# microsoft/hyperspace

Measured on NVIDIA H100. Metric: createIndex rows/sec, higher is better.
Workload: dtype int64

## Files before the change

### hyperspace_b200/csrc/radix_sort.cu

```cuda
#include <cmath>

#include "device_utils.cuh"
#include "kernels.h"

namespace hs {

struct SortChunk {
  uint32_t seg;
  uint32_t tile_begin, tile_end;
};

namespace {

constexpr int kThreads = 512;
constexpr int kWarps = kThreads / 32;
constexpr int kItems = kSortTile / kThreads;
constexpr int kWarpRows = kSortTile / kWarps;
constexpr int kChunkTiles = 128;
constexpr int kHistThreads = 256;

struct DigitShift {
  int shift;
  __device__ __forceinline__ uint32_t operator()(uint64_t key, uint32_t) const { return (uint32_t)(key >> shift) & 255u; }
};
struct DigitTable {
  const uint8_t* table;
  __device__ __forceinline__ uint32_t operator()(uint64_t, uint32_t val) const { return table[val]; }
};

struct SrcPairs {
  const uint64_t* __restrict__ keys;
  const uint32_t* __restrict__ vals;
  __device__ __forceinline__ void load(uint64_t p, uint64_t& k, uint32_t& v) const {
    k = keys[p];
    v = vals[p];
  }
};
template <int TYPE>
struct SrcRaw {
  const void* __restrict__ raw;
  __device__ __forceinline__ void load(uint64_t p, uint64_t& k, uint32_t& v) const {
    const uint64_t r = (TYPE == HS_TYPE_INT64 || TYPE == HS_TYPE_DOUBLE) ? ((const uint64_t*)raw)[p]
                                                                          : (uint64_t)((const uint32_t*)raw)[p];
    k = sort_encode(TYPE, r);
    v = (uint32_t)p;
  }
};

template <typename Src, typename Digit>
__global__ void __launch_bounds__(kHistThreads) k_sort_hist(const SortTile* __restrict__ tiles, Src src, Digit digit,
                                                         uint32_t* __restrict__ tile_hist) {
  __shared__ uint32_t s_hist[256];
  s_hist[threadIdx.x] = 0;
  __syncthreads();
  const SortTile t = tiles[blockIdx.x];
  for (uint32_t i = threadIdx.x; i < t.count; i += kHistThreads) {
    uint64_t k;
    uint32_t v;
    src.load(t.start + i, k, v);
    atomicAdd(&s_hist[digit(k, v)], 1u);
  }
  __syncthreads();
  tile_hist[(size_t)blockIdx.x * 256 + threadIdx.x] = s_hist[threadIdx.x];
}

__global__ void __launch_bounds__(256) k_seg_chunk_sums(const SortChunk* __restrict__ chunks,
                                                         const uint32_t* __restrict__ tile_hist,
                                                         uint32_t* __restrict__ chunk_sums) {
  const SortChunk c = chunks[blockIdx.x];
  uint32_t s = 0;
  for (uint32_t t = c.tile_begin; t < c.tile_end; t++) s += tile_hist[(size_t)t * 256 + threadIdx.x];
  chunk_sums[(size_t)blockIdx.x * 256 + threadIdx.x] = s;
}

__global__ void __launch_bounds__(256) k_seg_scan(const uint32_t* __restrict__ seg_chunk_begin,
                                                   const uint64_t* __restrict__ seg_start,
                                                   uint32_t* __restrict__ chunk_sums, uint32_t* __restrict__ digit_base) {
  __shared__ uint32_t warp_sums[40];
  const uint32_t seg = blockIdx.x;
  const uint32_t c0 = seg_chunk_begin[seg], c1 = seg_chunk_begin[seg + 1];
  uint32_t tot = 0;
  for (uint32_t c = c0; c < c1; c++) {
    const uint32_t v = chunk_sums[(size_t)c * 256 + threadIdx.x];
    chunk_sums[(size_t)c * 256 + threadIdx.x] = tot;
    tot += v;
  }
  const uint32_t dbase = block_exclusive_scan(tot, warp_sums, nullptr) + (uint32_t)seg_start[seg];
  if (digit_base) digit_base[(size_t)seg * 256 + threadIdx.x] = dbase;
  for (uint32_t c = c0; c < c1; c++) chunk_sums[(size_t)c * 256 + threadIdx.x] += dbase;
}

__global__ void __launch_bounds__(1024) k_seg_apply(const SortChunk* __restrict__ chunks,
                                                     const uint32_t* __restrict__ tile_hist,
                                                     uint32_t* __restrict__ tile_dst,
                                                     const uint32_t* __restrict__ chunk_sums) {
  __shared__ uint32_t s_group[4][256];
  const SortChunk c = chunks[blockIdx.x];
  const uint32_t d = threadIdx.x & 255, g = threadIdx.x >> 8;
  const uint32_t n = c.tile_end - c.tile_begin;
  const uint32_t per = (n + 3) / 4;
  const uint32_t t0 = c.tile_begin + min(g * per, n), t1 = c.tile_begin + min((g + 1) * per, n);
  uint32_t s = 0;
#pragma unroll 8
  for (uint32_t t = t0; t < t1; t++) s += tile_hist[(size_t)t * 256 + d];
  s_group[g][d] = s;
  __syncthreads();
  uint32_t run = chunk_sums[(size_t)blockIdx.x * 256 + d];
  for (uint32_t gg = 0; gg < g; gg++) run += s_group[gg][d];
#pragma unroll 8
  for (uint32_t t = t0; t < t1; t++) {
    const uint32_t v = tile_hist[(size_t)t * 256 + d];
    tile_dst[(size_t)t * 256 + d] = run;
    run += v;
  }
}

template <int W, int I, bool kGuard, typename Bin>
__device__ __forceinline__ uint32_t rank_tile(uint16_t (&cnt)[W][256], uint32_t* warp_sums, Bin bin, uint32_t count,
                                              uint32_t (&rank)[I]) {
  const uint32_t warp = threadIdx.x >> 5, lane = threadIdx.x & 31;
  const unsigned lt = (1u << lane) - 1;
  uint16_t* wcnt = cnt[warp];
#pragma unroll
  for (int j = 0; j < I; j++) {
    rank[j] = 0;
    if (!kGuard || warp * (I * 32) + j * 32 < count) {
      const uint32_t b = bin(j);
      const unsigned peers = match_any_full<8>(b);
      const uint32_t before = __popc(peers & lt);
      const uint32_t pre = wcnt[b];
      __syncwarp();
      if (before == 0) wcnt[b] = (uint16_t)(pre + __popc(peers));
      __syncwarp();
      rank[j] = pre + before;
    }
  }
  __syncthreads();
  uint32_t total = 0;
  if (threadIdx.x < 256) {
#pragma unroll
    for (int w = 0; w < W; w++) total += cnt[w][threadIdx.x];
  }
  const uint32_t start = block_exclusive_scan(total, warp_sums, nullptr);
  if (threadIdx.x < 256) {
    uint32_t run = start;
#pragma unroll
    for (int w = 0; w < W; w++) {
      const uint16_t c = cnt[w][threadIdx.x];
      cnt[w][threadIdx.x] = (uint16_t)run;
      run += c;
    }
  }
  return start;
}

struct ScatterShared {
  uint64_t keys[kSortTile];
  uint32_t vals[kSortTile];
  uint16_t cnt[kWarps][256];
  uint32_t out_adj[256];
  uint32_t warp_sums[40];
};

template <typename Src, typename Digit>
__global__ void __launch_bounds__(kThreads, 2) k_sort_scatter(const SortTile* __restrict__ tiles, Src src, Digit digit,
                                                               const uint32_t* __restrict__ tile_dst,
                                                               uint64_t* __restrict__ out_keys,
                                                               uint32_t* __restrict__ out_vals) {
  extern __shared__ __align__(16) uint8_t smem_raw[];
  ScatterShared& sm = *reinterpret_cast<ScatterShared*>(smem_raw);
  const uint32_t warp = threadIdx.x >> 5, lane = threadIdx.x & 31;
  {
    uint32_t* z = reinterpret_cast<uint32_t*>(&sm.cnt[0][0]);
#pragma unroll
    for (int i = 0; i < kWarps * 256 / 2 / kThreads; i++) z[threadIdx.x + i * kThreads] = 0;
  }
  const SortTile t = tiles[blockIdx.x];
  uint32_t dst0 = 0;
  if (threadIdx.x < 256) dst0 = tile_dst[(size_t)blockIdx.x * 256 + threadIdx.x];
  const uint32_t first = warp * kWarpRows + lane;
  const uint64_t p0 = t.start + first;
  uint64_t k[kItems];
  uint32_t v[kItems];
  uint32_t bin[kItems];
#pragma unroll
  for (int j = 0; j < kItems; j++) {
    const bool a = first + j * 32 < t.count;
    k[j] = ~0ull;
    v[j] = 0;
    if (a) src.load(p0 + j * 32, k[j], v[j]);
    bin[j] = a ? digit(k[j], v[j]) : 255u;
  }
  __syncthreads();
  uint32_t rank[kItems];
  const uint32_t start = rank_tile<kWarps, kItems, false>(sm.cnt, sm.warp_sums, [&](int j) { return bin[j]; }, 0, rank);
  if (threadIdx.x < 256) sm.out_adj[threadIdx.x] = dst0 - start;
  __syncthreads();
  const uint16_t* cnt = sm.cnt[warp];
#pragma unroll
  for (int j = 0; j < kItems; j++) {
    const uint32_t pos = cnt[bin[j]] + rank[j];
    sm.keys[pos] = k[j];
    sm.vals[pos] = v[j];
  }
  __syncthreads();
#pragma unroll
  for (int j = 0; j < kItems; j++) {
    const uint32_t i = threadIdx.x + j * kThreads;
    if (i < t.count) {
      const uint64_t key = sm.keys[i];
      const uint32_t val = sm.vals[i];
      const uint32_t dst = sm.out_adj[digit(key, val)] + i;
      out_keys[dst] = key;
      out_vals[dst] = val;
    }
  }
}

constexpr uint32_t kFixMaxRun = 64;
__global__ void __launch_bounds__(256) k_fix_runs(const SortTile* __restrict__ tiles, const uint64_t* __restrict__ seg_start,
                                                   uint64_t* __restrict__ keys, uint32_t* __restrict__ vals,
                                                   uint64_t high_mask, uint64_t low_mask, uint32_t max_run,
                                                   uint32_t* __restrict__ flag) {
  __shared__ uint64_t s_key[kSortTile + 2];
  __shared__ uint16_t s_heads[kSortTile / 2], s_len[kSortTile / 2];
  const SortTile t = tiles[blockIdx.x];
  const uint64_t segb = seg_start[t.seg], sege = seg_start[t.seg + 1];
  const unsigned lane = threadIdx.x & 31, lt = (1u << lane) - 1;
  constexpr int kPer = kSortTile / 256;
  {
    uint64_t k[kPer];
#pragma unroll
    for (int j = 0; j < kPer; j++) {
      const uint32_t i = j * 256 + threadIdx.x;
      k[j] = i < t.count ? keys[t.start + i] : 0;
    }
#pragma unroll
    for (int j = 0; j < kPer; j++) s_key[1 + j * 256 + threadIdx.x] = k[j];
  }
  __syncthreads();
  if (threadIdx.x == 0) {
    const uint64_t flip = high_mask & (~high_mask + 1);
    s_key[0] = t.start > segb ? keys[t.start - 1] : (s_key[1] ^ flip);
    s_key[t.count + 1] = t.start + t.count < sege ? keys[t.start + t.count] : (s_key[t.count] ^ flip);
  }
  __syncthreads();
  const uint32_t wid = threadIdx.x >> 5;
  uint16_t* my_heads = s_heads + wid * (kSortTile / 16);
  uint16_t* my_len = s_len + wid * (kSortTile / 16);
  uint32_t my_n = 0;
#pragma unroll 4
  for (uint32_t i0 = 0; i0 < kSortTile; i0 += 256) {
    const uint32_t i = i0 + threadIdx.x;
    bool head = false;
    if (i < t.count) {
      const uint64_t kh = s_key[1 + i] & high_mask;
      head = (s_key[i] & high_mask) != kh && (s_key[2 + i] & high_mask) == kh;
    }
    const unsigned m = __ballot_sync(0xffffffffu, head);
    if (head) my_heads[my_n + __popc(m & lt)] = (uint16_t)i;
    my_n += __popc(m);
  }
  __syncwarp();
  for (uint32_t e = lane; e < my_n; e += 32) {
    const uint32_t i = my_heads[e];
    const uint64_t* sk = s_key + 1 + i;
    const uint64_t kh = sk[0] & high_mask;
    uint32_t len = 1;
    while (i + len < t.count && len <= max_run && (sk[len] & high_mask) == kh) len++;
    const bool crosses = i + len == t.count && (sk[len] & high_mask) == kh;
    my_len[e] = crosses ? (uint16_t)0xffffu : (uint16_t)len;
  }
  __syncthreads();
  for (uint32_t e = lane; e < my_n; e += 32) {
    const uint32_t i = my_heads[e];
    const uint64_t p = t.start + i;
    uint64_t* sk = s_key + 1 + i;
    const uint64_t kh = sk[0] & high_mask;
    uint32_t len = my_len[e];
    if (len == 0xffffu) {
      len = t.count - i;
      uint64_t q = p + len;
      while (q < sege && q - p <= max_run && (keys[q] & high_mask) == kh) q++;
      const uint32_t glen = (uint32_t)(q - p);
      if (glen > max_run) {
        *flag = 1;
        continue;
      }
      for (uint32_t a = 1; a < glen; a++) {
        const uint64_t ka = keys[p + a];
        const uint32_t va = vals[p + a];
        const uint64_t la = ka & low_mask;
        uint32_t b = a;
        while (b > 0 && (keys[p + b - 1] & low_mask) > la) {
          keys[p + b] = keys[p + b - 1];
          vals[p + b] = vals[p + b - 1];
          b--;
        }
        if (b != a) {
          keys[p + b] = ka;
          vals[p + b] = va;
        }
      }
      continue;
    }
    if (len > max_run) {
      *flag = 1;
      continue;
    }
    for (uint32_t a = 1; a < len; a++) {
      const uint64_t ka = sk[a];
      const uint64_t la = ka & low_mask;
      uint32_t b = a;
      while (b > 0 && (sk[b - 1] & low_mask) > la) b--;
      if (b == a) continue;
      const uint32_t va = vals[p + a];
      for (uint32_t c = a; c > b; c--) {
        const uint64_t kc = sk[c - 1];
        sk[c] = kc;
        keys[p + c] = kc;
        vals[p + c] = vals[p + c - 1];
      }
      sk[b] = ka;
      keys[p + b] = ka;
      vals[p + b] = va;
    }
  }
}

constexpr int kLocalSortCap = 12288;
struct LocalSortItem {
  uint32_t start, count;
};
constexpr int kLocalThreads = 1024;
constexpr int kLocalWarps = kLocalThreads / 32;
constexpr int kLocalItems = kLocalSortCap / kLocalThreads;
constexpr int kLocalWarpRows = kLocalSortCap / kLocalWarps;
constexpr uint32_t kLocalMaxRun = 64;
static_assert(kLocalSortCap % kLocalThreads == 0 && kLocalSortCap <= 65536, "slot numbers are 16-bit");

struct LocalShared {
  uint64_t keys[kLocalSortCap];
  uint32_t vals[kLocalSortCap];
  uint16_t slot[kLocalSortCap];
  uint16_t cnt[kLocalWarps][256];
  uint32_t warp_sums[40];
  unsigned long long or_bits, and_bits;
  uint32_t long_run;
};

__device__ __forceinline__ void local_pass(LocalShared& sm, uint32_t count, int shift) {
  const uint32_t warp = threadIdx.x >> 5, lane = threadIdx.x & 31;
  {
    uint32_t* z = reinterpret_cast<uint32_t*>(&sm.cnt[0][0]);
#pragma unroll
    for (int i = 0; i < kLocalWarps * 256 / 2 / kLocalThreads; i++) z[threadIdx.x + i * kLocalThreads] = 0;
  }
  const uint32_t first = warp * kLocalWarpRows + lane;
  uint32_t slot_bin[kLocalItems], rank[kLocalItems];
#pragma unroll
  for (int j = 0; j < kLocalItems; j++) {
    const uint32_t pos = first + j * 32;
    const uint32_t s = pos < count ? sm.slot[pos] : pos;
    slot_bin[j] = s << 8 | (pos < count ? (uint32_t)(sm.keys[s] >> shift) & 255u : 255u);
  }
  __syncthreads();
  rank_tile<kLocalWarps, kLocalItems, true>(sm.cnt, sm.warp_sums, [&](int j) { return slot_bin[j] & 255u; }, count, rank);
  __syncthreads();
  const uint16_t* cnt = sm.cnt[warp];
#pragma unroll
  for (int j = 0; j < kLocalItems; j++)
    if (warp * kLocalWarpRows + j * 32 < count) sm.slot[cnt[slot_bin[j] & 255u] + rank[j]] = (uint16_t)(slot_bin[j] >> 8);
  __syncthreads();
}

template <typename Src>
__global__ void __launch_bounds__(kLocalThreads, 1) k_local_sort(const LocalSortItem* __restrict__ items, Src src,
                                                                 uint64_t* __restrict__ out_keys,
                                                                 uint32_t* __restrict__ out_vals) {
  extern __shared__ __align__(16) uint8_t smem_raw[];
  LocalShared& sm = *reinterpret_cast<LocalShared*>(smem_raw);
  const LocalSortItem it = items[blockIdx.x];
  const uint32_t count = it.count;
  if (threadIdx.x == 0) {
    sm.or_bits = 0;
    sm.and_bits = ~0ull;
    sm.long_run = 0;
  }
  uint64_t k_or = 0, k_and = ~0ull;
  constexpr int kHalf = kLocalItems / 2;
#pragma unroll 1
  for (int h = 0; h < 2; h++) {
    uint64_t k[kHalf];
    uint32_t v[kHalf];
#pragma unroll
    for (int j = 0; j < kHalf; j++) {
      const uint32_t i = (h * kHalf + j) * kLocalThreads + threadIdx.x;
      if (i < count) src.load((uint64_t)it.start + i, k[j], v[j]);
    }
#pragma unroll
    for (int j = 0; j < kHalf; j++) {
      const uint32_t i = (h * kHalf + j) * kLocalThreads + threadIdx.x;
      if (i < count) {
        sm.keys[i] = k[j];
        sm.vals[i] = v[j];
        sm.slot[i] = (uint16_t)i;
        k_or |= k[j];
        k_and &= k[j];
      }
    }
  }
#pragma unroll
  for (int o = 16; o > 0; o >>= 1) {
    k_or |= __shfl_xor_sync(0xffffffffu, k_or, o);
    k_and &= __shfl_xor_sync(0xffffffffu, k_and, o);
  }
  __syncthreads();
  if ((threadIdx.x & 31) == 0) {
    atomicOr(&sm.or_bits, k_or);
    atomicAnd(&sm.and_bits, k_and);
  }
  __syncthreads();
  const uint64_t varying = sm.or_bits ^ sm.and_bits;
  if (varying != 0) {
    const int top = 63 - __clzll((long long)varying);
    int pbits = 1;
    while ((1u << pbits) < 2 * count) pbits++;
    const int ndig = (min(pbits, top + 1) + 7) / 8;
    const int low = max(0, top + 1 - 8 * ndig);
    for (int d = ndig - 1; d >= 0; d--) {
      const int shift = max(0, top + 1 - 8 * (d + 1));
      if ((varying >> shift) & 0xff) local_pass(sm, count, shift);
    }
    const uint64_t high_mask = ~0ull << low;
    if (varying & ~high_mask) {
      for (uint32_t i = threadIdx.x; i < count; i += kLocalThreads) {
        const uint64_t kh = sm.keys[sm.slot[i]] & high_mask;
        if (i > 0 && (sm.keys[sm.slot[i - 1]] & high_mask) == kh) continue;
        if (i + 1 >= count || (sm.keys[sm.slot[i + 1]] & high_mask) != kh) continue;
        uint32_t len = 2;
        while (i + len < count && len <= kLocalMaxRun && (sm.keys[sm.slot[i + len]] & high_mask) == kh) len++;
        if (len > kLocalMaxRun) {
          sm.long_run = 1;
          continue;
        }
        uint16_t* s = sm.slot + i;
        for (uint32_t a = 1; a < len; a++) {
          const uint16_t sa = s[a];
          const uint64_t ka = sm.keys[sa];
          uint32_t b = a;
          while (b > 0 && sm.keys[s[b - 1]] > ka) {
            s[b] = s[b - 1];
            b--;
          }
          s[b] = sa;
        }
      }
      __syncthreads();
      if (sm.long_run) {
        for (uint32_t i = threadIdx.x; i < count; i += kLocalThreads) sm.slot[i] = (uint16_t)i;
        __syncthreads();
        for (int shift = 0; shift < 64; shift += 8)
          if ((varying >> shift) & 0xff) local_pass(sm, count, shift);
      }
    }
  }
  __syncthreads();
#pragma unroll
  for (int j = 0; j < kLocalItems; j++) {
    const uint32_t i = j * kLocalThreads + threadIdx.x;
    if (i < count) {
      const uint32_t s = sm.slot[i];
      out_keys[(uint64_t)it.start + i] = sm.keys[s];
      out_vals[(uint64_t)it.start + i] = sm.vals[s];
    }
  }
}

template <typename Src>
void launch_local_sort(hs_ctx* ctx, const std::vector<LocalSortItem>& items, Src src, uint64_t* out_keys,
                       uint32_t* out_vals) {
  if (items.empty()) return;
  Buf<LocalSortItem> d_items(ctx, items.size());
  copy_h2d(ctx, d_items.get(), items.data(), items.size() * sizeof(LocalSortItem));
  static DeviceOnce attr_once;
  bool& attr = attr_once(ctx->device);
  if (!attr) {
    HS_CUDA(cudaFuncSetAttribute(k_local_sort<Src>, cudaFuncAttributeMaxDynamicSharedMemorySize, (int)sizeof(LocalShared)));
    attr = true;
  }
  KernelScope _ks(ctx, "k_local_sort");
  k_local_sort<Src><<<(unsigned)items.size(), kLocalThreads, sizeof(LocalShared), ctx->stream>>>(d_items.get(), src,
                                                                                                 out_keys, out_vals);
  HS_LAUNCH_CHECK(ctx);
}

template <typename Src, typename Digit>
void run_hist(hs_ctx* ctx, SortPlan* plan, Src src, Digit digit, uint32_t* digit_base) {
  {
    KernelScope _ks(ctx, "k_sort_hist");
    k_sort_hist<Src, Digit><<<(unsigned)plan->ntiles, kHistThreads, 0, ctx->stream>>>(plan->tiles.get(), src, digit,
                                                                                 plan->tile_hist.get());
    HS_LAUNCH_CHECK(ctx);
  }
  KernelScope _ks(ctx, "k_seg_scan");
  k_seg_chunk_sums<<<(unsigned)plan->nchunks, 256, 0, ctx->stream>>>(plan->chunks.get(), plan->tile_hist.get(),
                                                                     plan->chunk_sums.get());
  HS_LAUNCH_CHECK(ctx);
  k_seg_scan<<<(unsigned)plan->nseg, 256, 0, ctx->stream>>>(plan->seg_chunk_begin.get(), plan->seg_start.get(),
                                                            plan->chunk_sums.get(), digit_base);
  HS_LAUNCH_CHECK(ctx);
}

template <typename Src, typename Digit>
void run_scatter(hs_ctx* ctx, SortPlan* plan, Src src, Digit digit, uint64_t* out_keys, uint32_t* out_vals) {
  {
    KernelScope _ks(ctx, "k_seg_scan");
    k_seg_apply<<<(unsigned)plan->nchunks, 1024, 0, ctx->stream>>>(plan->chunks.get(), plan->tile_hist.get(),
                                                                   plan->tile_dst.get(), plan->chunk_sums.get());
    HS_LAUNCH_CHECK(ctx);
  }
  static DeviceOnce attr_once;
  bool& attr = attr_once(ctx->device);
  if (!attr) {
    HS_CUDA(cudaFuncSetAttribute(k_sort_scatter<Src, Digit>, cudaFuncAttributeMaxDynamicSharedMemorySize,
                                 (int)sizeof(ScatterShared)));
    attr = true;
  }
  KernelScope _ks(ctx, "k_sort_scatter");
  k_sort_scatter<Src, Digit><<<(unsigned)plan->ntiles, kThreads, sizeof(ScatterShared), ctx->stream>>>(
      plan->tiles.get(), src, digit, plan->tile_dst.get(), out_keys, out_vals);
  HS_LAUNCH_CHECK(ctx);
}

template <typename Src, typename Digit>
void run_pass(hs_ctx* ctx, SortPlan* plan, Src src, Digit digit, SortedRows* s) {
  run_hist(ctx, plan, src, digit, nullptr);
  run_scatter(ctx, plan, src, digit, s->keys_buf[s->cur ^ 1].get(), s->perm_buf[s->cur ^ 1].get());
  s->cur ^= 1;
}

template <typename F>
void with_raw_source(const KeyColumn& raw, F&& f) {
  switch (raw.type) {
    case HS_TYPE_INT32: f(SrcRaw<HS_TYPE_INT32>{raw.data}); break;
    case HS_TYPE_INT64: f(SrcRaw<HS_TYPE_INT64>{raw.data}); break;
    case HS_TYPE_FLOAT: f(SrcRaw<HS_TYPE_FLOAT>{raw.data}); break;
    case HS_TYPE_DOUBLE: f(SrcRaw<HS_TYPE_DOUBLE>{raw.data}); break;
    default: fail(HS_EUNSUPPORTED, "sort: key type %d", raw.type);
  }
}

void lsd_passes(hs_ctx* ctx, SortPlan* plan, SortedRows* s, uint64_t bits, const KeyColumn* raw) {
  if (plan->ntiles == 0) return;
  bool first = raw != nullptr;
  for (int pass = 0; pass < 8; pass++) {
    if (((bits >> (pass * 8)) & 0xff) == 0) continue;
    const DigitShift digit{pass * 8};
    if (first)
      with_raw_source(*raw, [&](auto src) { run_pass(ctx, plan, src, digit, s); });
    else
      run_pass(ctx, plan, SrcPairs{s->keys(), s->perm()}, digit, s);
    first = false;
  }
  if (first) fail(HS_EINVAL, "sort: raw first-pass source given but no pass ran");
}

void local_sort_segments(hs_ctx* ctx, const SortPlan& plan, const KeyColumn& raw, SortedRows* s) {
  std::vector<LocalSortItem> items;
  for (int g = 0; g < plan.nseg; g++) {
    const uint64_t n = plan.h_seg_start[g + 1] - plan.h_seg_start[g];
    if (n) items.push_back(LocalSortItem{(uint32_t)plan.h_seg_start[g], (uint32_t)n});
  }
  with_raw_source(raw, [&](auto src) { launch_local_sort(ctx, items, src, s->keys(), s->perm()); });
}

bool msd_local_sort(hs_ctx* ctx, SortPlan* plan, const KeyColumn& raw, int shift, SortedRows* s) {
  if (plan->ntiles == 0) return false;
  const size_t nsub = (size_t)plan->nseg * 256;
  Buf<uint32_t> d_base(ctx, nsub);
  const DigitShift digit{shift};
  with_raw_source(raw, [&](auto src) { run_hist(ctx, plan, src, digit, d_base.get()); });
  std::vector<uint32_t> base(nsub + 1);
  copy_d2h(ctx, base.data(), d_base.get(), nsub * 4);
  sync_stream(ctx);
  base[nsub] = (uint32_t)plan->n;
  std::vector<LocalSortItem> items;
  for (int g = 0; g < plan->nseg; g++) {
    LocalSortItem cur{base[(size_t)g * 256], 0};
    for (size_t d = (size_t)g * 256; d < (size_t)(g + 1) * 256; d++) {
      const uint32_t sz = base[d + 1] - base[d];
      if (sz > (uint32_t)kLocalSortCap) return false;
      if (cur.count + sz > (uint32_t)kLocalSortCap) {
        items.push_back(cur);
        cur = LocalSortItem{base[d], 0};
      }
      cur.count += sz;
    }
    if (cur.count) items.push_back(cur);
  }
  uint64_t* keys_alt = s->keys_buf[s->cur ^ 1].get();
  uint32_t* perm_alt = s->perm_buf[s->cur ^ 1].get();
  with_raw_source(raw, [&](auto src) { run_scatter(ctx, plan, src, digit, keys_alt, perm_alt); });
  launch_local_sort(ctx, items, SrcPairs{keys_alt, perm_alt}, s->keys(), s->perm());
  return true;
}

}

__global__ void k_build_tiles(const uint64_t* __restrict__ seg_start, const uint32_t* __restrict__ seg_tile_begin,
                              SortTile* __restrict__ tiles) {
  const uint32_t s = blockIdx.x;
  const uint64_t b = seg_start[s], e = seg_start[s + 1];
  const uint32_t t0 = seg_tile_begin[s], nt = seg_tile_begin[s + 1] - t0;
  for (uint32_t i = threadIdx.x; i < nt; i += blockDim.x) {
    const uint64_t p = b + (uint64_t)i * kSortTile;
    tiles[t0 + i] = SortTile{s, (uint32_t)min((uint64_t)kSortTile, e - p), p};
  }
}

void build_sort_plan(hs_ctx* ctx, const uint64_t* seg_offsets, int nseg, SortPlan* plan) {
  std::vector<uint32_t> stb(nseg + 1), scb(nseg + 1);
  std::vector<uint64_t> sstart(nseg + 1);
  std::vector<SortChunk> chunks;
  uint64_t ntiles = 0;
  for (int s = 0; s < nseg; s++) {
    stb[s] = (uint32_t)ntiles;
    sstart[s] = seg_offsets[s];
    ntiles += ceil_div(seg_offsets[s + 1] - seg_offsets[s], (uint64_t)kSortTile);
    scb[s] = (uint32_t)chunks.size();
    for (uint32_t t = stb[s]; t < ntiles; t += kChunkTiles)
      chunks.push_back(SortChunk{(uint32_t)s, t, (uint32_t)std::min<uint64_t>(t + kChunkTiles, ntiles)});
  }
  stb[nseg] = (uint32_t)ntiles;
  sstart[nseg] = seg_offsets[nseg];
  scb[nseg] = (uint32_t)chunks.size();
  if (seg_offsets[nseg] >= (1ull << 32)) fail(HS_EUNSUPPORTED, "more than 2^32-1 rows per GPU per call");
  plan->n = (int64_t)seg_offsets[nseg];
  plan->ntiles = (int64_t)ntiles;
  plan->nseg = nseg;
  plan->nchunks = (int64_t)chunks.size();
  plan->tiles.alloc(ctx, std::max<size_t>(1, ntiles));
  plan->seg_tile_begin.alloc(ctx, stb.size());
  plan->seg_start.alloc(ctx, sstart.size());
  plan->tile_hist.alloc(ctx, std::max<size_t>(1, ntiles) * 256);
  plan->tile_dst.alloc(ctx, std::max<size_t>(1, ntiles) * 256);
  plan->chunks.alloc(ctx, std::max<size_t>(1, chunks.size()));
  plan->seg_chunk_begin.alloc(ctx, scb.size());
  plan->chunk_sums.alloc(ctx, std::max<size_t>(1, chunks.size()) * 256);
  copy_h2d(ctx, plan->seg_tile_begin.get(), stb.data(), stb.size() * 4);
  copy_h2d(ctx, plan->seg_start.get(), sstart.data(), sstart.size() * 8);
  if (!chunks.empty()) copy_h2d(ctx, plan->chunks.get(), chunks.data(), chunks.size() * sizeof(SortChunk));
  copy_h2d(ctx, plan->seg_chunk_begin.get(), scb.data(), scb.size() * 4);
  if (nseg > 0 && ntiles > 0) {
    k_build_tiles<<<nseg, 256, 0, ctx->stream>>>(plan->seg_start.get(), plan->seg_tile_begin.get(), plan->tiles.get());
    HS_LAUNCH_CHECK(ctx);
  }
  plan->h_seg_tile_begin = std::move(stb);
  plan->h_seg_start = std::move(sstart);
}

void sort_rows(hs_ctx* ctx, SortPlan* plan, const KeyColumn* cols, int ncols, const unsigned long long* last_or_and,
               bool may_defer, SortedRows* out) {
  const int64_t nrows = plan->n;
  for (auto& b : out->keys_buf) b.alloc(ctx, std::max<int64_t>(1, nrows));
  for (auto& b : out->perm_buf) b.alloc(ctx, std::max<int64_t>(1, nrows));
  out->cur = 0;
  out->queued = false;
  out->resort_bits = 0;
  Buf<unsigned long long> d_or_and(ctx, 2);
  unsigned long long or_and[2] = {0, 0};
  auto reduce = [&](auto launch) {
    const unsigned long long init[2] = {0ull, ~0ull};
    copy_h2d(ctx, d_or_and.get(), init, sizeof init);
    launch(d_or_and.get());
    copy_d2h(ctx, or_and, d_or_and.get(), sizeof or_and);
    sync_stream(ctx);
  };
  uint64_t max_seg = 1;
  for (int g = 0; g < plan->nseg; g++) max_seg = std::max<uint64_t>(max_seg, plan->h_seg_start[g + 1] - plan->h_seg_start[g]);
  int want_bytes = 2;
  while (want_bytes < 8 && (double)max_seg / std::pow(256.0, want_bytes) > 0.5) want_bytes++;
  const bool lsd_only = getenv("HS_LSD_SORT") != nullptr;
  for (int k = ncols - 1; k >= 0; k--) {
    const KeyColumn& kc = cols[k];
    const bool from_raw = k == ncols - 1 && kc.type >= HS_TYPE_INT32 && kc.type <= HS_TYPE_DOUBLE;
    if (k == ncols - 1 && !from_raw) launch_iota_u32(ctx, out->perm(), nrows);
    if (kc.type == HS_TYPE_STRING) {
      auto sort_piece = [&](int piece) {
        reduce([&](unsigned long long* d) {
          launch_string_piece_keys(ctx, (const uint64_t*)kc.data, out->perm(), nrows, piece, out->keys(), d);
        });
        lsd_passes(ctx, plan, out, or_and[0] ^ or_and[1], nullptr);
      };
      sort_piece(-1);
      const unsigned long long len_or = or_and[0];
      for (int piece = (int)((len_or + 7) / 8) - 1; piece >= 0; piece--) sort_piece(piece);
    } else {
      if (from_raw && last_or_and) {
        or_and[0] = last_or_and[0];
        or_and[1] = last_or_and[1];
      } else {
        reduce([&](unsigned long long* d) {
          launch_encode_keys(ctx, kc.data, kc.type, from_raw ? nullptr : out->perm(), nrows, from_raw ? nullptr : out->keys(), d);
        });
      }
      const uint64_t varying = nrows ? (or_and[0] ^ or_and[1]) : 0;
      int nbytes = 0, lowest_high_byte = 0;
      for (int b = 7, seen = 0; b >= 0; b--)
        if ((varying >> (8 * b)) & 0xff) {
          nbytes++;
          if (++seen == want_bytes) lowest_high_byte = b;
        }
      const KeyColumn* raw = from_raw ? &kc : nullptr;
      if (from_raw && varying == 0) {
        launch_iota_u32(ctx, out->perm(), nrows);
        launch_encode_keys(ctx, kc.data, kc.type, nullptr, nrows, out->keys(), d_or_and.get());
        raw = nullptr;
      }
      const bool defer = may_defer && ncols == 1 && !kc.valid;
      bool local = false;
      if (raw && !kc.valid && !lsd_only) {
        if (max_seg <= (uint64_t)kLocalSortCap) {
          local_sort_segments(ctx, *plan, kc, out);
          local = true;
        } else if (nbytes > 2 && max_seg <= (uint64_t)(0.85 * 256 * kLocalSortCap)) {
          local = msd_local_sort(ctx, plan, kc, std::max(0, 63 - __builtin_clzll(varying) - 7), out);
        }
      }
      if (local) {
        out->queued = defer;
      } else if (nbytes > want_bytes) {
        const uint64_t high_mask = ~0ull << (8 * lowest_high_byte);
        lsd_passes(ctx, plan, out, varying & high_mask, raw);
        Buf<uint32_t> d_gave_up(ctx, 1);
        fill_bytes(ctx, d_gave_up.get(), 0, 4);
        {
          KernelScope _ks(ctx, "k_fix_runs");
          k_fix_runs<<<(unsigned)plan->ntiles, 256, 0, ctx->stream>>>(plan->tiles.get(), plan->seg_start.get(), out->keys(),
                                                                      out->perm(), high_mask, ~high_mask, kFixMaxRun,
                                                                      d_gave_up.get());
          HS_LAUNCH_CHECK(ctx);
        }
        out->gave_up = 0;
        out->resort_bits = varying;
        out->queued_at = ctx->sync_count;
        out->queued = true;
        copy_d2h(ctx, &out->gave_up, d_gave_up.get(), 4);
        if (!defer) settle_sorted_rows(ctx, plan, out);
      } else {
        lsd_passes(ctx, plan, out, varying, raw);
      }
    }
    if (kc.valid && plan->ntiles)
      run_pass(ctx, plan, SrcPairs{out->keys(), out->perm()}, DigitTable{kc.valid}, out);
  }
}

bool settle_sorted_rows(hs_ctx* ctx, SortPlan* plan, SortedRows* s) {
  const uint64_t bits = s->resort_bits;
  s->queued = false;
  s->resort_bits = 0;
  if (bits == 0) return false;
  if (ctx->sync_count <= s->queued_at) sync_stream(ctx);
  if (!s->gave_up) return false;
  lsd_passes(ctx, plan, s, bits, nullptr);
  return true;
}

}
```

Baseline: 7.955 billion.

## Make local sort persistent with L2 bulk prefetch of next segment

Converts k_local_sort into a persistent kernel with one block per SM looping over items, and uses cp.async.bulk.prefetch.L2 to pull the next item's keys into L2 while the current one sorts. It also loads all items in one pass instead of two halves, skips the slot indirection on the first radix pass, and replaces the strided run-detection loop with warp-shuffle head detection. The aim is to hide global load latency and cut launch/tail effects. In exchange it serializes items per SM, which loses the overlap that multiple resident blocks would otherwise give, and it adds register pressure from the full-width load arrays.

Measured after the change: 8.028 billion (median of 6 runs). About the same (+0.9%).

```diff
diff --git a/hyperspace_b200/csrc/radix_sort.cu b/hyperspace_b200/csrc/radix_sort.cu
--- a/hyperspace_b200/csrc/radix_sort.cu
+++ b/hyperspace_b200/csrc/radix_sort.cu
@@ -28,6 +28,11 @@
   __device__ __forceinline__ uint32_t operator()(uint64_t, uint32_t val) const { return table[val]; }
 };
 
+__device__ __forceinline__ void prefetch_l2(const void* p, uint64_t bytes) {
+  const uint64_t a = (uint64_t)p, lo = (a + 15) & ~15ull, hi = (a + bytes) & ~15ull;
+  if (hi > lo) asm volatile("cp.async.bulk.prefetch.L2.global [%0], %1;" ::"l"(lo), "r"((uint32_t)(hi - lo)) : "memory");
+}
+
 struct SrcPairs {
   const uint64_t* __restrict__ keys;
   const uint32_t* __restrict__ vals;
@@ -35,15 +40,22 @@
     k = keys[p];
     v = vals[p];
   }
+  __device__ __forceinline__ void prefetch(uint64_t p, uint32_t n) const {
+    prefetch_l2(keys + p, (uint64_t)n * sizeof(uint64_t));
+    prefetch_l2(vals + p, (uint64_t)n * sizeof(uint32_t));
+  }
 };
 template <int TYPE>
 struct SrcRaw {
+  static constexpr int kWidth = (TYPE == HS_TYPE_INT64 || TYPE == HS_TYPE_DOUBLE) ? 8 : 4;
   const void* __restrict__ raw;
   __device__ __forceinline__ void load(uint64_t p, uint64_t& k, uint32_t& v) const {
-    const uint64_t r = (TYPE == HS_TYPE_INT64 || TYPE == HS_TYPE_DOUBLE) ? ((const uint64_t*)raw)[p]
-                                                                          : (uint64_t)((const uint32_t*)raw)[p];
+    const uint64_t r = kWidth == 8 ? ((const uint64_t*)raw)[p] : (uint64_t)((const uint32_t*)raw)[p];
     k = sort_encode(TYPE, r);
     v = (uint32_t)p;
+  }
+  __device__ __forceinline__ void prefetch(uint64_t p, uint32_t n) const {
+    prefetch_l2((const uint8_t*)raw + p * kWidth, (uint64_t)n * kWidth);
   }
 };
 
@@ -349,7 +361,7 @@
   uint32_t long_run;
 };
 
-__device__ __forceinline__ void local_pass(LocalShared& sm, uint32_t count, int shift) {
+__device__ __forceinline__ void local_pass(LocalShared& sm, uint32_t count, int shift, bool identity) {
   const uint32_t warp = threadIdx.x >> 5, lane = threadIdx.x & 31;
   {
     uint32_t* z = reinterpret_cast<uint32_t*>(&sm.cnt[0][0]);
@@ -361,7 +373,7 @@
 #pragma unroll
   for (int j = 0; j < kLocalItems; j++) {
     const uint32_t pos = first + j * 32;
-    const uint32_t s = pos < count ? sm.slot[pos] : pos;
+    const uint32_t s = pos < count && !identity ? sm.slot[pos] : pos;
     slot_bin[j] = s << 8 | (pos < count ? (uint32_t)(sm.keys[s] >> shift) & 255u : 255u);
   }
   __syncthreads();
@@ -375,105 +387,133 @@
 }
 
 template <typename Src>
-__global__ void __launch_bounds__(kLocalThreads, 1) k_local_sort(const LocalSortItem* __restrict__ items, Src src,
+__global__ void __launch_bounds__(kLocalThreads, 1) k_local_sort(const LocalSortItem* __restrict__ items,
+                                                                 uint32_t nitems, Src src,
                                                                  uint64_t* __restrict__ out_keys,
                                                                  uint32_t* __restrict__ out_vals) {
   extern __shared__ __align__(16) uint8_t smem_raw[];
   LocalShared& sm = *reinterpret_cast<LocalShared*>(smem_raw);
-  const LocalSortItem it = items[blockIdx.x];
-  const uint32_t count = it.count;
-  if (threadIdx.x == 0) {
-    sm.or_bits = 0;
-    sm.and_bits = ~0ull;
-    sm.long_run = 0;
-  }
-  uint64_t k_or = 0, k_and = ~0ull;
-  constexpr int kHalf = kLocalItems / 2;
-#pragma unroll 1
-  for (int h = 0; h < 2; h++) {
-    uint64_t k[kHalf];
-    uint32_t v[kHalf];
-#pragma unroll
-    for (int j = 0; j < kHalf; j++) {
-      const uint32_t i = (h * kHalf + j) * kLocalThreads + threadIdx.x;
-      if (i < count) src.load((uint64_t)it.start + i, k[j], v[j]);
-    }
-#pragma unroll
-    for (int j = 0; j < kHalf; j++) {
-      const uint32_t i = (h * kHalf + j) * kLocalThreads + threadIdx.x;
+  for (uint32_t b = blockIdx.x; b < nitems; b += gridDim.x) {
+    const LocalSortItem it = items[b];
+    const uint32_t count = it.count;
+    if (threadIdx.x == 0) {
+      if (b + gridDim.x < nitems) {
+        const LocalSortItem next = items[b + gridDim.x];
+        src.prefetch(next.start, next.count);
+      }
+      sm.or_bits = 0;
+      sm.and_bits = ~0ull;
+      sm.long_run = 0;
+    }
+    uint64_t k_or = 0, k_and = ~0ull;
+    {
+      uint64_t k[kLocalItems];
+      uint32_t v[kLocalItems];
+#pragma unroll
+      for (int j = 0; j < kLocalItems; j++) {
+        const uint32_t i = j * kLocalThreads + threadIdx.x;
+        k[j] = 0;
+        v[j] = 0;
+        if (i < count) src.load((uint64_t)it.start + i, k[j], v[j]);
+      }
+#pragma unroll
+      for (int j = 0; j < kLocalItems; j++) {
+        const uint32_t i = j * kLocalThreads + threadIdx.x;
+        if (i < count) {
+          sm.keys[i] = k[j];
+          sm.vals[i] = v[j];
+          sm.slot[i] = (uint16_t)i;
+          k_or |= k[j];
+          k_and &= k[j];
+        }
+      }
+    }
+#pragma unroll
+    for (int o = 16; o > 0; o >>= 1) {
+      k_or |= __shfl_xor_sync(0xffffffffu, k_or, o);
+      k_and &= __shfl_xor_sync(0xffffffffu, k_and, o);
+    }
+    __syncthreads();
+    if ((threadIdx.x & 31) == 0) {
+      atomicOr(&sm.or_bits, k_or);
+      atomicAnd(&sm.and_bits, k_and);
+    }
+    __syncthreads();
+    const uint64_t varying = sm.or_bits ^ sm.and_bits;
+    if (varying != 0) {
+      const int top = 63 - __clzll((long long)varying);
+      int pbits = 1;
+      while ((1u << pbits) < 2 * count) pbits++;
+      const int ndig = (min(pbits, top + 1) + 7) / 8;
+      const int low = max(0, top + 1 - 8 * ndig);
+      bool identity = true;
+      for (int d = ndig - 1; d >= 0; d--) {
+        const int shift = max(0, top + 1 - 8 * (d + 1));
+        if ((varying >> shift) & 0xff) {
+          local_pass(sm, count, shift, identity);
+          identity = false;
+        }
+      }
+      const uint64_t high_mask = ~0ull << low;
+      if (varying & ~high_mask) {
+        const uint32_t lane = threadIdx.x & 31;
+        uint32_t heads = 0;
+#pragma unroll
+        for (int j = 0; j < kLocalItems; j++) {
+          const uint32_t i = j * kLocalThreads + threadIdx.x;
+          const uint64_t kh = i < count ? sm.keys[sm.slot[i]] & high_mask : 0;
+          uint64_t prev = __shfl_up_sync(0xffffffffu, kh, 1), next = __shfl_down_sync(0xffffffffu, kh, 1);
+          if (lane == 0 && i > 0 && i <= count) prev = sm.keys[sm.slot[i - 1]] & high_mask;
+          if (lane == 31 && i + 1 < count) next = sm.keys[sm.slot[i + 1]] & high_mask;
+          const bool head = i + 1 < count && (i == 0 || prev != kh) && next == kh;
+          heads |= (uint32_t)head << j;
+        }
+        while (heads) {
+          const uint32_t i = (uint32_t)(__ffs(heads) - 1) * kLocalThreads + threadIdx.x;
+          heads &= heads - 1;
+          const uint64_t kh = sm.keys[sm.slot[i]] & high_mask;
+          uint32_t len = 2;
+          while (i + len < count && len <= kLocalMaxRun && (sm.keys[sm.slot[i + len]] & high_mask) == kh) len++;
+          if (len > kLocalMaxRun) {
+            sm.long_run = 1;
+            continue;
+          }
+          uint16_t* s = sm.slot + i;
+          for (uint32_t a = 1; a < len; a++) {
+            const uint16_t sa = s[a];
+            const uint64_t ka = sm.keys[sa];
+            uint32_t b = a;
+            while (b > 0 && sm.keys[s[b - 1]] > ka) {
+              s[b] = s[b - 1];
+              b--;
+            }
+            s[b] = sa;
+          }
+        }
+        __syncthreads();
+        if (sm.long_run) {
+          for (uint32_t i = threadIdx.x; i < count; i += kLocalThreads) sm.slot[i] = (uint16_t)i;
+          __syncthreads();
+          bool identity = true;
+          for (int shift = 0; shift < 64; shift += 8)
+            if ((varying >> shift) & 0xff) {
+              local_pass(sm, count, shift, identity);
+              identity = false;
+            }
+        }
+      }
+    }
+    __syncthreads();
+#pragma unroll
+    for (int j = 0; j < kLocalItems; j++) {
+      const uint32_t i = j * kLocalThreads + threadIdx.x;
       if (i < count) {
-        sm.keys[i] = k[j];
-        sm.vals[i] = v[j];
-        sm.slot[i] = (uint16_t)i;
-        k_or |= k[j];
-        k_and &= k[j];
-      }
-    }
-  }
-#pragma unroll
-  for (int o = 16; o > 0; o >>= 1) {
-    k_or |= __shfl_xor_sync(0xffffffffu, k_or, o);
-    k_and &= __shfl_xor_sync(0xffffffffu, k_and, o);
-  }
-  __syncthreads();
-  if ((threadIdx.x & 31) == 0) {
-    atomicOr(&sm.or_bits, k_or);
-    atomicAnd(&sm.and_bits, k_and);
-  }
-  __syncthreads();
-  const uint64_t varying = sm.or_bits ^ sm.and_bits;
-  if (varying != 0) {
-    const int top = 63 - __clzll((long long)varying);
-    int pbits = 1;
-    while ((1u << pbits) < 2 * count) pbits++;
-    const int ndig = (min(pbits, top + 1) + 7) / 8;
-    const int low = max(0, top + 1 - 8 * ndig);
-    for (int d = ndig - 1; d >= 0; d--) {
-      const int shift = max(0, top + 1 - 8 * (d + 1));
-      if ((varying >> shift) & 0xff) local_pass(sm, count, shift);
-    }
-    const uint64_t high_mask = ~0ull << low;
-    if (varying & ~high_mask) {
-      for (uint32_t i = threadIdx.x; i < count; i += kLocalThreads) {
-        const uint64_t kh = sm.keys[sm.slot[i]] & high_mask;
-        if (i > 0 && (sm.keys[sm.slot[i - 1]] & high_mask) == kh) continue;
-        if (i + 1 >= count || (sm.keys[sm.slot[i + 1]] & high_mask) != kh) continue;
-        uint32_t len = 2;
-        while (i + len < count && len <= kLocalMaxRun && (sm.keys[sm.slot[i + len]] & high_mask) == kh) len++;
-        if (len > kLocalMaxRun) {
-          sm.long_run = 1;
-          continue;
-        }
-        uint16_t* s = sm.slot + i;
-        for (uint32_t a = 1; a < len; a++) {
-          const uint16_t sa = s[a];
-          const uint64_t ka = sm.keys[sa];
-          uint32_t b = a;
-          while (b > 0 && sm.keys[s[b - 1]] > ka) {
-            s[b] = s[b - 1];
-            b--;
-          }
-          s[b] = sa;
-        }
-      }
-      __syncthreads();
-      if (sm.long_run) {
-        for (uint32_t i = threadIdx.x; i < count; i += kLocalThreads) sm.slot[i] = (uint16_t)i;
-        __syncthreads();
-        for (int shift = 0; shift < 64; shift += 8)
-          if ((varying >> shift) & 0xff) local_pass(sm, count, shift);
-      }
-    }
-  }
-  __syncthreads();
-#pragma unroll
-  for (int j = 0; j < kLocalItems; j++) {
-    const uint32_t i = j * kLocalThreads + threadIdx.x;
-    if (i < count) {
-      const uint32_t s = sm.slot[i];
-      out_keys[(uint64_t)it.start + i] = sm.keys[s];
-      out_vals[(uint64_t)it.start + i] = sm.vals[s];
-    }
+        const uint32_t s = sm.slot[i];
+        out_keys[(uint64_t)it.start + i] = sm.keys[s];
+        out_vals[(uint64_t)it.start + i] = sm.vals[s];
+      }
+    }
+    __syncthreads();
   }
 }
 
@@ -489,9 +529,10 @@
     HS_CUDA(cudaFuncSetAttribute(k_local_sort<Src>, cudaFuncAttributeMaxDynamicSharedMemorySize, (int)sizeof(LocalShared)));
     attr = true;
   }
+  const unsigned grid = (unsigned)std::min<size_t>(items.size(), (size_t)ctx->sm_count);
   KernelScope _ks(ctx, "k_local_sort");
-  k_local_sort<Src><<<(unsigned)items.size(), kLocalThreads, sizeof(LocalShared), ctx->stream>>>(d_items.get(), src,
-                                                                                                 out_keys, out_vals);
+  k_local_sort<Src><<<grid, kLocalThreads, sizeof(LocalShared), ctx->stream>>>(d_items.get(), (uint32_t)items.size(), src,
+                                                                               out_keys, out_vals);
   HS_LAUNCH_CHECK(ctx);
 }
 
```
